# wangg12/mx-DeepIM

Measured on AMD Instinct MI355X. Metric: pose-refinements/sec (4 iters, 480x640), higher is better.
Workload: dtype f32

## Files before the change

### mx-deepim_amd/csrc/common.h

```cpp
#pragma once
#include <hip/hip_runtime.h>
#include <cstdarg>
#include <cstdio>
#include <cstdint>
#include <utility>

#include "../../include/deepim_hip.h"

namespace dim {

constexpr int kWave = 64;

char* err_buf();
int set_err(int code, const char* fmt, ...);

inline hipStream_t as_stream(void* s) { return reinterpret_cast<hipStream_t>(s); }

inline int check_launch(const char* what) {
  hipError_t e = hipGetLastError();
  if (e != hipSuccess) return set_err(DIM_ERR_LAUNCH, "%s: %s", what, hipGetErrorString(e));
  return DIM_OK;
}

inline int ceil_div(long a, long b) { return (int)((a + b - 1) / b); }
// ... 165 lines not shown
  for (int g = 1; g <= 8; g <<= 1) {
    if (count % g || wtile_lds_bytes(g, Q) > 65536) break;
    if (best == 0 || (long)outer * (count / g) >= 2048 || count / best > 65535) best = g;
  }
  return (best && count / best <= 65535 && outer <= 65535) ? best : 0;
}
template <bool TO_PACKED, typename PT>
inline void wtile_launch(const WTileArgs& a, int gx, int gy, hipStream_t st) {
  hipLaunchKernelGGL((weight_tile_kernel<TO_PACKED, PT>), dim3(gx, gy), dim3(256), wtile_lds_bytes(a.G, a.Q), st, a);
}
#endif

int conv2d_unpack_weight_slabs(const float* w_packed, int nslab, long slab_stride, float* w_oihw, int Cout, int CoutPad, int Cin, int KH, int KW,
                               float scale, int accumulate, void* stream);

struct WGemmArgs {
  const float* V;
  const float* U;
  float* M;
  int T, K, Cout, P;
  int nch;
  int NTN;
  int per, rem;
  unsigned v_bytes, u_bytes, m_bytes;
  FastDiv d_nch, d_P, d_NTN, d_MT;
  int G, BM, BN, tile;
  int MT;
  int plane_major;
  int dbg_plain;
  int wide_flush;
  const void* U3;
  unsigned u3_bytes;
  int split;
};
inline long wino_packed_with_split(long u_floats) { return u_floats + (u_floats * 3 + 1) / 2; }
int wino_split_weights(float* U, long chunks, int Cout, hipStream_t st);
void wino_set_split(int on);
int wino_get_split();
bool wino_gemm_split_has(int tile);
int wino_gemm_split_slots(int tile);
int wino_gemm_split_run(const WGemmArgs& a, hipStream_t st);
int wino_gemm_plan(WGemmArgs* plan, const float* V, const float* U, float* M, int T, int K, int Cout, int P, int tile);
int wino_gemm_run(const WGemmArgs& plan, bool zeroed, hipStream_t st);

#ifdef __HIPCC__
struct WCur {
  int ch, p, nt, mt;
};
__device__ __forceinline__ WCur wcur_decode(int chunk, const WGemmArgs& a) {
  WCur c;
  const unsigned item = fastdiv((unsigned)chunk, a.d_nch);
  c.ch = chunk - (int)item * a.nch;
  if (a.plane_major) {
    const unsigned t = fastdiv(item, a.d_NTN);
    c.nt = (int)(item - t * a.NTN);
    const unsigned p = fastdiv(t, a.d_MT);
    c.mt = (int)(t - p * a.MT);
    c.p = (int)p;
  } else {
    const unsigned t = fastdiv(item, a.d_P);
    c.p = (int)(item - t * a.P);
    const unsigned mt = fastdiv(t, a.d_NTN);
    c.nt = (int)(t - mt * a.NTN);
    c.mt = (int)mt;
  }
  return c;
}
__device__ __forceinline__ int wg_xcd_contiguous(int b, int G) {
  const int x = b & 7, j = b >> 3, q = G >> 3, r = G & 7;
  return (x < r ? x * (q + 1) : r * (q + 1) + (x - r) * q) + j;
}
__device__ __forceinline__ int wg_first_chunk(int w, const WGemmArgs& a) { return w * a.per + min(w, a.rem); }
__device__ __forceinline__ void wino_gemm_zero_tile(const WGemmArgs& a, int w) {
  const WCur c = wcur_decode(wg_first_chunk(w, a), a);
  if (c.ch == 0) return;
  const int ldc = a.P * a.Cout;
  float* base = a.M + (long)c.mt * a.BM * ldc + c.p * a.Cout + c.nt * a.BN;
  const int rows = min(a.BM, a.T - c.mt * a.BM);
  const int q = a.BN / 4;
  for (int idx = threadIdx.x; idx < rows * q; idx += 256) {
    const int r = idx / q, c4 = idx - r * q;
    *reinterpret_cast<float4*>(base + (long)r * ldc + c4 * 4) = make_float4(0.f, 0.f, 0.f, 0.f);
  }
}
#endif

}

#define DIM_REQUIRE(cond, ...)                                   \
  do {                                                           \
    if (!(cond)) return dim::set_err(DIM_ERR_ARG, __VA_ARGS__);  \
  } while (0)
```

### mx-deepim_amd/csrc/wino_gemm.hip

```cpp
#include <cstdlib>

#include "common.h"

namespace dim {

typedef float f32x16 __attribute__((ext_vector_type(16)));

__device__ __forceinline__ void wcur_advance(WCur& c, const WGemmArgs& a) {
  if (++c.ch == a.nch) {
    c.ch = 0;
    if (a.plane_major) {
      if (++c.nt == a.NTN) {
        c.nt = 0;
        if (++c.mt == a.MT) {
          c.mt = 0;
          ++c.p;
        }
      }
    } else if (++c.p == a.P) {
      c.p = 0;
      if (++c.nt == a.NTN) {
        c.nt = 0;
        ++c.mt;
      }
    }
  }
}
template <int BM, int BN, int WM, int WN>
__global__ __launch_bounds__(WM * WN * 64) __attribute__((amdgpu_waves_per_eu(BN == 256 || BM == 160 ? 2 : (BM == 96 ? 3 : 4), 8))) void wino_gemm_kernel(WGemmArgs a) {
  constexpr int BK = 32;
  constexpr int NT = WM * WN * 64;
  constexpr int RP = NT / 8;
  constexpr int LDK = BK + 4;
  constexpr int TM = BM / WM / 32;
  constexpr int TN = BN / WN / 32;
  constexpr int NSTG = BM / RP;
  constexpr int kTrLd = 32, kTrFloats = 16 * kTrLd;
  constexpr bool kWide = !(BM == 128 && BN == 128);
  static_assert(BM % RP == 0 && NSTG >= 2 && NSTG <= 5, "two to five staging loads per thread");

  extern __shared__ __attribute__((aligned(16))) float smem[];
  float* sA = smem;
  float* sTr = smem + 2 * BM * LDK;

  const int tid = threadIdx.x;
  const int lane = tid & 63;
  const int wave = tid >> 6;
  const int wm = wave / WN, wn = wave % WN;
  const int q = tid & 7;
  const int srow = tid >> 3;
  const int frow = lane & 31;
  const int khalf = lane >> 5;

  const int wg = a.plane_major ? wg_xcd_contiguous(blockIdx.x, a.G) : (int)blockIdx.x;
  const int c_begin = wg_first_chunk(wg, a);
  const int c_end = wg_first_chunk(wg + 1, a);

  const int RS = a.P * a.K;
  const int a_voff0 = (srow * RS + q * 4) * 4;
  const int a_vstep = RP * RS * 4;
  const __amdgpu_buffer_rsrc_t rv = __builtin_amdgcn_make_buffer_rsrc(const_cast<float*>(a.V), 0, a.v_bytes, 0x00020000);
  const __amdgpu_buffer_rsrc_t ru = __builtin_amdgcn_make_buffer_rsrc(const_cast<float*>(a.U), 0, a.u_bytes, 0x00020000);
  const __amdgpu_buffer_rsrc_t rm = __builtin_amdgcn_make_buffer_rsrc(a.M, 0, a.m_bytes, 0x00020000);
  const int wchunk_bytes = a.Cout * BK * 4;

  WCur L = wcur_decode(c_begin, a), Bc = L, C = L;

  float4 ra0, ra1, ra2, ra3, ra4;
#define W_LOAD_CHUNK(PF_OK)                                                            \
  {                                                                                    \
    const bool pf = (PF_OK);                                                           \
    const int mb = L.mt * BM;                                                          \
    const int soff = (int)((unsigned)(mb * RS + L.p * a.K + L.ch * BK) * 4u);          \
    ra0 = buf_load16_nt(rv, (pf && mb + srow < a.T) ? a_voff0 : -1, soff);             \
    ra1 = buf_load16_nt(rv, (pf && mb + srow + RP < a.T) ? a_voff0 + a_vstep : -1, soff);        \
    if constexpr (NSTG > 2) ra2 = buf_load16_nt(rv, (pf && mb + srow + 2 * RP < a.T) ? a_voff0 + 2 * a_vstep : -1, soff); \
    if constexpr (NSTG > 3) ra3 = buf_load16_nt(rv, (pf && mb + srow + 3 * RP < a.T) ? a_voff0 + 3 * a_vstep : -1, soff); \
    if constexpr (NSTG > 4) ra4 = buf_load16_nt(rv, (pf && mb + srow + 4 * RP < a.T) ? a_voff0 + 4 * a_vstep : -1, soff); \
    wcur_advance(L, a);                                                                \
  }
#define W_STORE_CHUNK(BUF)                                                             \
  {                                                                                    \
    float* dA = sA + (BUF) * BM * LDK;                                                 \
    *reinterpret_cast<float4*>(dA + srow * LDK + q * 4) = ra0;                         \
    *reinterpret_cast<float4*>(dA + (srow + RP) * LDK + q * 4) = ra1;                  \
    if constexpr (NSTG > 2) *reinterpret_cast<float4*>(dA + (srow + 2 * RP) * LDK + q * 4) = ra2; \
    if constexpr (NSTG > 3) *reinterpret_cast<float4*>(dA + (srow + 3 * RP) * LDK + q * 4) = ra3; \
    if constexpr (NSTG > 4) *reinterpret_cast<float4*>(dA + (srow + 4 * RP) * LDK + q * 4) = ra4; \
  }

  f32x16 acc[TM][TN];
#pragma unroll
  for (int i = 0; i < TM; ++i)
#pragma unroll
    for (int j = 0; j < TN; ++j)
#pragma unroll
      for (int r = 0; r < 16; ++r) acc[i][j][r] = 0.f;

  const int a_off = (wm * (BM / WM) + frow) * LDK + 4 * khalf;
  float4 fa[2][TM];
#define W_FRAG_READ(IDX, PA, S)                                                                                        \
  {                                                                                                                    \
    _Pragma("unroll") for (int i = 0; i < TM; ++i) fa[IDX][i] = *reinterpret_cast<const float4*>((PA) + 32 * i * LDK + 8 * (S)); \
  }
  float4 fbq[2][4][TN];
  const int bf_voff = ((wn * (BN / WN) + frow) * BK + 4 * khalf) * 4;
#define W_LOAD_BFRAG(SET, VALID)                                                                                       \
  {                                                                                                                    \
    const int bsoff = (VALID) ? (Bc.p * a.nch + Bc.ch) * wchunk_bytes + Bc.nt * BN * BK * 4 : 0;                        \
    _Pragma("unroll") for (int g = 0; g < 4; ++g) _Pragma("unroll") for (int j = 0; j < TN; ++j)                        \
      fbq[SET][g][j] = buf_load16(ru, bf_voff + (32 * j * BK + 8 * g) * 4, bsoff);                                      \
    wcur_advance(Bc, a);                                                                                               \
  }
#define W_MFMA_GROUP(IDX, SET, G)                                                                                      \
  {                                                                                                                    \
    __builtin_amdgcn_sched_barrier(0);                                                                                 \
    _Pragma("unroll") for (int i = 0; i < TM; ++i) _Pragma("unroll") for (int j = 0; j < TN; ++j) {                     \
      acc[i][j] = __builtin_amdgcn_mfma_f32_32x32x2f32(fa[IDX][i].x, fbq[SET][G][j].x, acc[i][j], 0, 0, 0);             \
      acc[i][j] = __builtin_amdgcn_mfma_f32_32x32x2f32(fa[IDX][i].y, fbq[SET][G][j].y, acc[i][j], 0, 0, 0);             \
      acc[i][j] = __builtin_amdgcn_mfma_f32_32x32x2f32(fa[IDX][i].z, fbq[SET][G][j].z, acc[i][j], 0, 0, 0);             \
      acc[i][j] = __builtin_amdgcn_mfma_f32_32x32x2f32(fa[IDX][i].w, fbq[SET][G][j].w, acc[i][j], 0, 0, 0);             \
    }                                                                                                                  \
    __builtin_amdgcn_sched_barrier(0);                                                                                 \
  }

  const int ldc = a.P * a.Cout;
  const int o_row = wm * (BM / WM) + 4 * khalf;
  const int o_col = wn * (BN / WN) + frow;
  const int o_voff = (o_row * ldc + o_col) * 4;
  bool whole = C.ch == 0;
#define W_FLUSH_CHECK(KCUR)                                                                                            \
  {                                                                                                                    \
    const bool item_end = C.ch == a.nch - 1;                                                                           \
    if (item_end || (KCUR) == c_end - 1) {                                                                             \
      const int mb = C.mt * BM;                                                                                        \
      const int cb = C.p * a.Cout + C.nt * BN;                                                                         \
      const int lim = a.T - mb;                                                                                        \
      int ov = o_voff, orow = o_row;  \
      asm volatile("" : "+v"(ov), "+v"(orow));                                                                         \
      const int soff = (int)((unsigned)(mb * ldc + cb) * 4u);                                                          \
      const bool plain = (whole && item_end) || a.dbg_plain;                                                           \
      if (kWide && plain && a.wide_flush) {                                                                            \
                                                        \
        float* sT = sTr + wave * kTrFloats;                                                                            \
        const int trow = lane >> 3, tc4 = (lane & 7) * 4;                                                              \
        _Pragma("unroll") for (int i = 0; i < TM; ++i) _Pragma("unroll") for (int j = 0; j < TN; ++j)                   \
          _Pragma("unroll") for (int h = 0; h < 2; ++h) {  \
            _Pragma("unroll") for (int r = 0; r < 8; ++r) sT[((r & 3) + 8 * (r >> 2) + 4 * khalf) * kTrLd + frow] = acc[i][j][8 * h + r]; \
            asm volatile("s_waitcnt lgkmcnt(0)" ::: "memory");                                                         \
             \
            const float4 t0 = *reinterpret_cast<const float4*>(sT + trow * kTrLd + tc4);                               \
            const float4 t1 = *reinterpret_cast<const float4*>(sT + (trow + 8) * kTrLd + tc4);                         \
            asm volatile("s_waitcnt lgkmcnt(0)" ::: "memory");                                                         \
            const int gr = wm * (BM / WM) + 32 * i + 16 * h + trow;                                                    \
            const int vo0 = (gr < lim) ? (gr * ldc + wn * (BN / WN) + 32 * j + tc4) * 4 : -1;                          \
            const int vo1 = (gr + 8 < lim) ? ((gr + 8) * ldc + wn * (BN / WN) + 32 * j + tc4) * 4 : -1;                \
            u32x4 u0, u1;                                                                                              \
            u0.x = __float_as_uint(t0.x); u0.y = __float_as_uint(t0.y); u0.z = __float_as_uint(t0.z); u0.w = __float_as_uint(t0.w); \
            u1.x = __float_as_uint(t1.x); u1.y = __float_as_uint(t1.y); u1.z = __float_as_uint(t1.z); u1.w = __float_as_uint(t1.w); \
            __builtin_amdgcn_raw_buffer_store_b128(u0, rm, vo0, soff, 2);                                              \
            __builtin_amdgcn_raw_buffer_store_b128(u1, rm, vo1, soff, 2);                                              \
            asm volatile("" ::: "memory");                                                                             \
          }                                                                                                            \
      } else                                                                                                           \
      _Pragma("unroll") for (int i = 0; i < TM; ++i) _Pragma("unroll") for (int j = 0; j < TN; ++j)                     \
        _Pragma("unroll") for (int r = 0; r < 16; ++r) {                                                               \
// ... 44 lines not shown
  }
#undef W_CHUNK_BODY
#undef W_FLUSH_CHECK
#undef W_MFMA_GROUP
#undef W_LOAD_BFRAG
#undef W_FRAG_READ
#undef W_STORE_CHUNK
#undef W_LOAD_CHUNK
}

__global__ __launch_bounds__(256) void wino_gemm_zero_kernel(WGemmArgs a) { wino_gemm_zero_tile(a, blockIdx.x + 1); }

static int g_wino_split = getenv("DIM_WINO_SPLIT") ? atoi(getenv("DIM_WINO_SPLIT")) : 1;
void wino_set_split(int on) { g_wino_split = on; }
int wino_get_split() { return g_wino_split; }
static int g_wino_cus = 0;
template <int BM, int BN, int WM, int WN>
static int wino_gemm_slots() {
  static int slots = 0;
  if (slots == 0) {
    int dev = 0, cus = 0, occ = 0;
    hipError_t e = hipGetDevice(&dev);
    if (e == hipSuccess) e = hipDeviceGetAttribute(&cus, hipDeviceAttributeMultiprocessorCount, dev);
    if (e == hipSuccess)
      e = hipOccupancyMaxActiveBlocksPerMultiprocessor(&occ, reinterpret_cast<const void*>(&wino_gemm_kernel<BM, BN, WM, WN>),
                                                       WM * WN * 64, (2 * BM * 36 + WM * WN * 512) * sizeof(float));
    if (e != hipSuccess || cus <= 0 || occ <= 0) return set_err(DIM_ERR_LAUNCH, "winograd gemm occupancy query: %s", hipGetErrorString(e));
    slots = cus * occ;
    g_wino_cus = cus;
  }
  return slots;
}

int wino_gemm_plan(WGemmArgs* plan, const float* V, const float* U, float* M, int T, int K, int Cout, int P, int tile) {
  if (tile == 5 && Cout % 256 != 0) tile = 4;
  if ((tile < 4 || tile > 7) || Cout % 128 != 0) tile = 3;
  const int BM = tile == 3 ? 64 : tile == 6 ? 160 : tile == 7 ? 96 : 128, BN = tile == 5 ? 256 : tile == 3 ? 64 : 128;
  DIM_REQUIRE(K % 32 == 0 && Cout % BN == 0 && T > 0, "winograd gemm: K %% 32 == 0 and Cout %% 64 == 0 required");
  const long MT = (T + BM - 1) / BM;
  const long items = MT * (Cout / BN) * P;
  DIM_REQUIRE(items * (K / 32) < (1L << 31) && (long)T * P * K * 4 < (1L << 32) && (long)T * P * Cout * 4 < (1L << 32) &&
                  (long)P * K * Cout * 4 < (1L << 31) && (long)BM * P * (K > Cout ? K : Cout) * 4 < (1L << 31),
              "winograd gemm: problem too large for 32-bit byte offsets (split the batch)");
  WGemmArgs a = {};
  a.V = V;
  a.U = U;
  a.M = M;
  a.T = T;
  a.K = K;
  a.Cout = Cout;
  a.P = P;
  a.nch = K / 32;
  a.NTN = Cout / BN;
  a.v_bytes = (unsigned)((long)T * P * K * 4);
  a.u_bytes = (unsigned)((long)P * K * Cout * 4);
  a.m_bytes = (unsigned)((long)T * P * Cout * 4);
  a.d_nch = make_fastdiv((unsigned)a.nch);
  a.d_P = make_fastdiv((unsigned)P);
  a.d_NTN = make_fastdiv((unsigned)a.NTN);
  a.MT = (int)MT;
  a.d_MT = make_fastdiv((unsigned)MT);
  static const int order = getenv("DIM_WINO_PLANE_MAJOR") ? atoi(getenv("DIM_WINO_PLANE_MAJOR")) : 1;
  a.plane_major = order;
  static const int dbg_plain = getenv("DIM_WINO_DBG_PLAIN") ? atoi(getenv("DIM_WINO_DBG_PLAIN")) : 0;
  a.dbg_plain = dbg_plain;
  static const int wide = getenv("DIM_WINO_WIDE_FLUSH") ? atoi(getenv("DIM_WINO_WIDE_FLUSH")) : 1;
  a.wide_flush = wide;
  a.BM = BM;
  a.BN = BN;
  a.tile = tile;
  a.split = g_wino_split && wino_gemm_split_has(tile) && (long)P * K * Cout * 6 < (1L << 31);
  a.U3 = U + (long)P * K * Cout;
  a.u3_bytes = (unsigned)((long)P * K * Cout * 6);
  if (a.split) a.plane_major = 1;
  const int slots = a.split ? wino_gemm_split_slots(tile) : tile == 5 ? wino_gemm_slots<128, 256, 2, 4>() : tile == 4 ? wino_gemm_slots<128, 128, 2, 4>()
                  : tile == 6 ? wino_gemm_slots<160, 128, 1, 4>() : tile == 7 ? wino_gemm_slots<96, 128, 1, 4>() : wino_gemm_slots<64, 64, 2, 2>();
  if (slots <= 0) return slots;
  a.G = items < slots ? (int)items : slots;
  static const int g_round = getenv("DIM_WINO_G_ROUND") ? atoi(getenv("DIM_WINO_G_ROUND")) : 1;
  if (g_wino_cus == 0) {
    int dev = 0;
    if (hipGetDevice(&dev) != hipSuccess || hipDeviceGetAttribute(&g_wino_cus, hipDeviceAttributeMultiprocessorCount, dev) != hipSuccess) g_wino_cus = 0;
  }
  if (g_round && g_wino_cus > 0 && a.G > g_wino_cus && a.G < slots) a.G = a.G / g_wino_cus * g_wino_cus;
  const long total = items * a.nch;
  a.per = (int)(total / a.G);
  a.rem = (int)(total % a.G);
  *plan = a;
  return DIM_OK;
}

template <int BM, int BN, int WM, int WN>
static int wino_gemm_launch(const WGemmArgs& a, hipStream_t st) {
  constexpr size_t lds = (2 * BM * 36 + WM * WN * 512) * sizeof(float);
  static_assert(lds <= 65536, "dynamic LDS of a plane-GEMM workgroup stays within 64 KB");
  hipLaunchKernelGGL((wino_gemm_kernel<BM, BN, WM, WN>), dim3(a.G), dim3(WM * WN * 64), lds, st, a);
  return check_launch("winograd_gemm");
}

int wino_gemm_run(const WGemmArgs& a, bool zeroed, hipStream_t st) {
  if (!zeroed && a.G > 1) hipLaunchKernelGGL(wino_gemm_zero_kernel, dim3(a.G - 1), dim3(256), 0, st, a);
  if (a.split) return wino_gemm_split_run(a, st);
  if (a.tile == 5) return wino_gemm_launch<128, 256, 2, 4>(a, st);
  if (a.tile == 4) return wino_gemm_launch<128, 128, 2, 4>(a, st);
  if (a.tile == 6) return wino_gemm_launch<160, 128, 1, 4>(a, st);
  if (a.tile == 7) return wino_gemm_launch<96, 128, 1, 4>(a, st);
  return wino_gemm_launch<64, 64, 2, 2>(a, st);
// ... 11 lines not shown
```

### mx-deepim_amd/csrc/wino_gemm_split.hip

```cpp
#include <cstdlib>

#include "common.h"

#ifndef DIM_SPLIT_EXP
#define DIM_SPLIT_EXP 0
#endif
#ifndef DIM_SPLIT_OPT
#define DIM_SPLIT_OPT 0
#endif

namespace dim {

typedef float f32x16 __attribute__((ext_vector_type(16)));
typedef float f32x4 __attribute__((ext_vector_type(4)));
typedef __bf16 bf16x8 __attribute__((ext_vector_type(8)));
typedef __bf16 bf16x4 __attribute__((ext_vector_type(4)));

struct Split4 {
  uint2 h, m, l;
};
__device__ __forceinline__ Split4 split3(const float4 v) {
  const f32x4 x = {v.x, v.y, v.z, v.w};
  const bf16x4 bh = __builtin_convertvector(x, bf16x4);
  const f32x4 r1 = x - __builtin_convertvector(bh, f32x4);
// ... 19 lines not shown
  const Split4 a = split3(src[0]), b = split3(src[1]);
  unsigned char* dst = U3 + (long)c * Cout * 192 + (long)(n >> 5) * 6144 + ((g >> 1) * 32 + (n & 31)) * 32 + (g & 1) * 16;
  *reinterpret_cast<uint4*>(dst) = make_uint4(a.h.x, a.h.y, b.h.x, b.h.y);
  *reinterpret_cast<uint4*>(dst + 2048) = make_uint4(a.m.x, a.m.y, b.m.x, b.m.y);
  *reinterpret_cast<uint4*>(dst + 4096) = make_uint4(a.l.x, a.l.y, b.l.x, b.l.y);
}

int wino_split_weights(float* U, long chunks, int Cout, hipStream_t st) {
  if (Cout % 32 != 0) return DIM_OK;
  const long total = chunks * Cout * 4;
  unsigned char* U3 = reinterpret_cast<unsigned char*>(U + chunks * Cout * 32);
  hipLaunchKernelGGL(wino_split_weights_kernel, dim3((unsigned)((total + 255) / 256)), dim3(256), 0, st, U, U3, total, Cout,
                     make_fastdiv((unsigned)Cout));
  return check_launch("winograd_split_weights");
}

#if DIM_SPLIT_EXP & 128
__device__ unsigned long long g_split_stamps[1024 * 8 * 11];
#endif
#if (DIM_SPLIT_EXP & 128) && defined(__HIP_DEVICE_COMPILE__)
#define S_STAMP(K)                                                                     \
  {                                                                                    \
    unsigned long long t_;                                                             \
    __builtin_amdgcn_sched_barrier(0);                                                 \
    asm volatile("s_memtime %0\n\ts_waitcnt lgkmcnt(0)" : "=s"(t_)::"memory");         \
    __builtin_amdgcn_sched_barrier(0);                                                 \
    seg[K] += t_ - tprev;                                                              \
    tprev = t_;                                                                        \
  }
#else
#define S_STAMP(K)
#endif

__device__ __forceinline__ void wscur_advance(WCur& c, const WGemmArgs& a) {
  if (++c.ch == a.nch) {
    c.ch = 0;
    if (++c.nt == a.NTN) {
      c.nt = 0;
      if (++c.mt == a.MT) {
        c.mt = 0;
        ++c.p;
      }
    }
  }
}

template <int BM, int WN>
__global__ __launch_bounds__(WN * 64) __attribute__((amdgpu_waves_per_eu(2, 2))) void wino_gemm_split_kernel(WGemmArgs a) {
  constexpr int BK = 32;
  constexpr int NT = WN * 64;
  constexpr int BN = 32 * WN;
  constexpr int TM = BM / 32;
  constexpr int RP = NT / 8;
  constexpr int NSTG = BM / RP;
  constexpr int PL = BM * 64;
  constexpr int kTrLd = 32, kTrFloats = 16 * kTrLd;
  constexpr int kMAux = ((DIM_SPLIT_OPT & 2) || BM == 96) ? 0 : 2;
  static_assert(BM % 32 == 0 && BM % RP == 0 && RP % 32 == 0 && NSTG >= 2 && NSTG <= 4, "two to four staging loads per thread");

  extern __shared__ __attribute__((aligned(16))) unsigned char smem_split[];
  unsigned char* sA = smem_split;
  float* sTr = reinterpret_cast<float*>(smem_split + 2 * 3 * PL);

  const int tid = threadIdx.x;
  const int lane = tid & 63;
  const int wave = tid >> 6;
  const int q = tid & 7;
  const int srow = tid >> 3;
  const int frow = lane & 31;
  const int khalf = lane >> 5;

  const int wg = wg_xcd_contiguous(blockIdx.x, a.G);
  const int c_begin = wg_first_chunk(wg, a);
  const int c_end = wg_first_chunk(wg + 1, a);

  const int RS = a.P * a.K;
  const int a_voff0 = (srow * RS + q * 4) * 4;
  const int a_vstep = RP * RS * 4;
  const __amdgpu_buffer_rsrc_t rv = __builtin_amdgcn_make_buffer_rsrc(const_cast<float*>(a.V), 0, a.v_bytes, 0x00020000);
  const __amdgpu_buffer_rsrc_t ru = __builtin_amdgcn_make_buffer_rsrc(const_cast<void*>(a.U3), 0, a.u3_bytes, 0x00020000);
  const __amdgpu_buffer_rsrc_t rm = __builtin_amdgcn_make_buffer_rsrc(a.M, 0, a.m_bytes, 0x00020000);
  const int wchunk_bytes = a.Cout * 192;

  WCur L = wcur_decode(c_begin, a), Bc = L, C = L;

  float4 rav[2][NSTG];
#define S_LOAD_PREP(PF_OK)                                                             \
  const bool l_pf = (PF_OK);                                                           \
  const int l_mb = L.mt * BM;                                                          \
  const int l_soff = (int)((unsigned)(l_mb * RS + L.p * a.K + L.ch * BK) * 4u);        \
  wscur_advance(L, a);
#define S_LOAD_ISSUE(RSET)                                                             \
  _Pragma("unroll") for (int ps = 0; ps < NSTG; ++ps)                                   \
    rav[RSET][ps] = buf_load16_nt(rv, (l_pf && l_mb + srow + ps * RP < a.T) ? a_voff0 + ps * a_vstep : -1, l_soff);
  const int st_off = srow * 64 + ((((q >> 1) ^ (srow >> 2)) & 3) << 4) + (q & 1) * 8;
#define S_STORE_ONE(DA, R, PASS)                                                       \
  {                                                                                    \
    const Split4 s = split3(R);                                                        \
    *reinterpret_cast<uint2*>((DA) + (PASS) * RP * 64) = s.h;                          \
    *reinterpret_cast<uint2*>((DA) + PL + (PASS) * RP * 64) = s.m;                     \
    *reinterpret_cast<uint2*>((DA) + 2 * PL + (PASS) * RP * 64) = s.l;                 \
  }
#define S_STORE_CHUNK(BUF, RSET)                                                       \
  {                                                                                    \
    unsigned char* dA = sA + (BUF) * 3 * PL + st_off;                                  \
    _Pragma("unroll") for (int ps = 0; ps < NSTG; ++ps) S_STORE_ONE(dA, rav[RSET][ps], ps) \
  }

  f32x16 acc[TM];
#pragma unroll
  for (int i = 0; i < TM; ++i)
#pragma unroll
    for (int r = 0; r < 16; ++r) acc[i][r] = 0.f;

  const int fr_off = frow * 64 + (((khalf ^ (frow >> 2)) & 3) << 4);
  bf16x8 fa[TM][3];
#define S_FRAG_READ(T, PA, S)                                                                                          \
  {                                                                                                                    \
    _Pragma("unroll") for (int i = 0; i < TM; ++i)                                                                      \
      fa[i][T] = *reinterpret_cast<const bf16x8*>((PA) + (T) * PL + i * 2048 + (fr_off ^ (32 * (S))));                 \
  }
  bf16x8 fb[2][3][2];
  const int bf_voff = wave * 6144 + frow * 32 + khalf * 16;
#define S_BFRAG_PREP(VALID)                                                                                            \
  const int b_soff = (VALID) ? (Bc.p * a.nch + Bc.ch) * wchunk_bytes + Bc.nt * BN * 192 : 0;                            \
  wscur_advance(Bc, a);
#define S_BFRAG_ISSUE(SET)                                                                                             \
  _Pragma("unroll") for (int t = 0; t < 3; ++t) _Pragma("unroll") for (int s = 0; s < 2; ++s) {                         \
    const float4 v = buf_load16(ru, bf_voff + (t * 2 + s) * 1024, b_soff);                                             \
    fb[SET][t][s] = __builtin_bit_cast(bf16x8, v);                                                                     \
  }
  static constexpr int kTA[2][6] = {{2, 0, 1, 1, 0, 0}, {2, 1, 1, 0, 0, 0}};
  static constexpr int kTB[2][6] = {{0, 2, 1, 0, 1, 0}, {0, 1, 0, 2, 1, 0}};
  f32x4 sp_x, sp_r;
  bf16x4 sp_h, sp_m, sp_l;

  const int ldc = a.P * a.Cout;
  const int o_row = 4 * khalf;
  const int o_col = wave * 32 + frow;
  const int o_voff = (o_row * ldc + o_col) * 4;
  bool whole = C.ch == 0;
#define S_FLUSH_CHECK(KCUR)                                                                                            \
  {                                                                                                                    \
    const bool item_end = C.ch == a.nch - 1;                                                                           \
    if (item_end || (KCUR) == c_end - 1) {                                                                             \
      const int mb = C.mt * BM;                                                                                        \
      const int cb = C.p * a.Cout + C.nt * BN;                                                                         \
      const int lim = a.T - mb;                                                                                        \
      int ov = o_voff, orow = o_row;                                                                                   \
      asm volatile("" : "+v"(ov), "+v"(orow));                                                                         \
      const int soff = (int)((unsigned)(mb * ldc + cb) * 4u);                                                          \
      const bool plain = (whole && item_end) || a.dbg_plain;                                                           \
      if (plain && a.wide_flush) {                                                                                     \
        float* sT = sTr + wave * kTrFloats;                                                                            \
        const int trow = lane >> 3, tc4 = (lane & 7) * 4;                                                              \
        _Pragma("unroll") for (int i = 0; i < TM; ++i) _Pragma("unroll") for (int h = 0; h < 2; ++h) {                  \
                \
          if constexpr (!(DIM_SPLIT_OPT & 16))                                                                         \
          _Pragma("unroll") for (int r = 0; r < 8; ++r) sT[((r & 3) + 8 * (r >> 2) + 4 * khalf) * kTrLd + frow] = acc[i][8 * h + r]; \
          float4 t0, t1;                                                                                               \
          if constexpr (DIM_SPLIT_OPT & 16) {                            \
            t0 = make_float4(acc[i][8 * h], acc[i][8 * h + 1], acc[i][8 * h + 2], acc[i][8 * h + 3]);                  \
            t1 = make_float4(acc[i][8 * h + 4], acc[i][8 * h + 5], acc[i][8 * h + 6], acc[i][8 * h + 7]);              \
          } else {                                                                                                     \
            t0 = *reinterpret_cast<const float4*>(sT + trow * kTrLd + tc4);                                            \
            t1 = *reinterpret_cast<const float4*>(sT + (trow + 8) * kTrLd + tc4);                                      \
          }                                                                                                            \
          const int gr = 32 * i + 16 * h + trow;                                                                       \
          const int vo0 = (gr < lim) ? (gr * ldc + wave * 32 + tc4) * 4 : -1;                                          \
          const int vo1 = (gr + 8 < lim) ? ((gr + 8) * ldc + wave * 32 + tc4) * 4 : -1;                                \
          u32x4 u0, u1;                                                                                                \
          u0.x = __float_as_uint(t0.x); u0.y = __float_as_uint(t0.y); u0.z = __float_as_uint(t0.z); u0.w = __float_as_uint(t0.w); \
          u1.x = __float_as_uint(t1.x); u1.y = __float_as_uint(t1.y); u1.z = __float_as_uint(t1.z); u1.w = __float_as_uint(t1.w); \
          if constexpr (DIM_SPLIT_OPT & 8) {                                             \
            if constexpr (!(DIM_SPLIT_OPT & 64)) asm volatile("" ::"v"(u0), "v"(u1));                                  \
          } else {                                                                                                     \
            __builtin_amdgcn_raw_buffer_store_b128(u0, rm, vo0, soff, kMAux);                                          \
// ... 188 lines not shown
```

### mx-deepim_amd/csrc/winograd.hip

```cpp
#include <cstdlib>

#include "common.h"

namespace dim {

__device__ __forceinline__ float4 f4add(float4 a, float4 b) { return make_float4(a.x + b.x, a.y + b.y, a.z + b.z, a.w + b.w); }
__device__ __forceinline__ float4 f4sub(float4 a, float4 b) { return make_float4(a.x - b.x, a.y - b.y, a.z - b.z, a.w - b.w); }

__global__ __launch_bounds__(256) void wino_input_kernel(const float* __restrict__ x, float* __restrict__ V, int N, int H, int W, int C,
                                                         int in_cstride, int th, int tw, FastDiv div_cq, FastDiv div_tw, FastDiv div_th) {
  const unsigned idx = blockIdx.x * 256u + threadIdx.x;
  const unsigned CQ = C >> 2;
  const unsigned T = (unsigned)N * th * tw;
  const unsigned t = fastdiv(idx, div_cq);
  if (t >= T) return;
  const unsigned cq = idx - t * CQ;
  const unsigned r = fastdiv(t, div_tw);
  const unsigned tx = t - r * tw;
  const unsigned n = fastdiv(r, div_th);
  const unsigned ty = r - n * th;
  const int y0 = 2 * (int)ty - 1, x0 = 2 * (int)tx - 1;
  const float* base = x + (long)n * H * W * in_cstride + cq * 4;
  float4 d[4][4];
#pragma unroll
// ... 89 lines not shown
    Gg[0][j] = g[j];
    Gg[1][j] = 0.5f * (g[j] + g[3 + j] + g[6 + j]);
    Gg[2][j] = 0.5f * (g[j] - g[3 + j] + g[6 + j]);
    Gg[3][j] = g[6 + j];
  }
  const long per_k = (long)Cin * Cout;
  float* o = wp + ((long)(ci >> 5) * Cout + co) * 32 + (ci & 31);
#pragma unroll
  for (int i = 0; i < 4; ++i) {
    o[(i * 4 + 0) * per_k] = Gg[i][0];
    o[(i * 4 + 1) * per_k] = 0.5f * (Gg[i][0] + Gg[i][1] + Gg[i][2]);
    o[(i * 4 + 2) * per_k] = 0.5f * (Gg[i][0] - Gg[i][1] + Gg[i][2]);
    o[(i * 4 + 3) * per_k] = Gg[i][2];
  }
}

constexpr int kWino4Vec = 2;

template <int VEC>
struct WinoVec {
  typedef float type __attribute__((ext_vector_type(VEC)));
};

#define DIM_WINO4_BT(O, D, S)                                                          \
  {                                                                                    \
    O[0 * S] = D[0] + 1.5f * D[1] - 2.f * D[2] - 1.5f * D[3] + D[4];                    \
    O[1 * S] = D[4] - D[1] - 2.5f * D[2] - 0.5f * D[3];                                 \
    O[2 * S] = D[4] + D[1] + 0.5f * D[2] - 2.5f * D[3];                                 \
    O[3 * S] = D[4] - 0.5f * D[1] - D[2] + 0.5f * D[3];                                 \
    O[4 * S] = D[4] + 2.f * D[1] - D[2] - 2.f * D[3];                                   \
    O[5 * S] = D[1] + 1.5f * D[2] - 2.f * D[3] - 1.5f * D[4] + D[5];                    \
  }

template <int VEC, int S>
__global__ __launch_bounds__(256) void wino4_input_kernel(const float* __restrict__ x, float* __restrict__ V, int N, int H, int W, int C,
                                                          int in_cstride, int th, int tw, FastDiv div_cq, FastDiv div_tw, FastDiv div_th,
                                                          unsigned nblk, WGemmArgs plan) {
#pragma clang fp contract(fast)
  typedef typename WinoVec<VEC>::type vf;
  if (blockIdx.x >= nblk) {
    wino_gemm_zero_tile(plan, (int)(blockIdx.x - nblk) + 1);
    return;
  }
  const unsigned idx = (unsigned)wg_xcd_contiguous((int)blockIdx.x, (int)nblk) * 256u + threadIdx.x;
  const unsigned CT = C * S * S;
  const unsigned CQ = CT / VEC;
  const unsigned T = (unsigned)N * th * tw;
  const unsigned t = fastdiv(idx, div_cq);
  if (t >= T) return;
  const unsigned cq = idx - t * CQ;
  const unsigned r = fastdiv(t, div_tw);
  const unsigned tx = t - r * tw;
  const unsigned n = fastdiv(r, div_th);
  const unsigned ty = r - n * th;
  const int y0 = 4 * (int)ty - 1, x0 = 4 * (int)tx - 1;
  const unsigned cc = cq * VEC;
  const unsigned ph = S == 1 ? 0u : (unsigned)(cc >= (unsigned)C) + (unsigned)(cc >= 2u * C) + (unsigned)(cc >= 3u * C);
  const int py = ph >> 1, px = ph & 1;
  const float* base = x + (long)n * H * W * in_cstride + (cc - ph * C);
  vf tmp[36];
#pragma unroll
  for (int b = 0; b < 6; ++b) {
    const int xx = S * (x0 + b) + px;
    const bool okx = (unsigned)xx < (unsigned)W;
    const int xc = okx ? xx : 0;
    vf d[6];
#pragma unroll
    for (int a = 0; a < 6; ++a) {
      const int yy = S * (y0 + a) + py;
      const bool ok = okx && (unsigned)yy < (unsigned)H;
      const int yc = (unsigned)yy < (unsigned)H ? yy : 0;
      vf v = *reinterpret_cast<const vf*>(base + ((long)yc * W + xc) * in_cstride);
      d[a] = ok ? v : (vf)(0.f);
    }
    vf* o = tmp + b;
    DIM_WINO4_BT(o, d, 6)
  }
  const long plane = CT;
  float* out = V + (long)t * 36 * CT + cc;
#pragma unroll
  for (int a = 0; a < 6; ++a) {
    vf o[6];
    const vf* d = tmp + 6 * a;
    DIM_WINO4_BT(o, d, 1)
#pragma unroll
    for (int b = 0; b < 6; ++b) __builtin_nontemporal_store(o[b], reinterpret_cast<vf*>(out + (a * 6 + b) * plane));
  }
}

#define DIM_WINO4_AT(O, M, S)                                       \
  {                                                                 \
    const vf s1 = M[1] + M[2], d1 = M[1] - M[2];                    \
    O[0 * S] = M[0] + s1 + M[3] + M[4];                             \
    O[1 * S] = d1 + 2.f * M[3] - 0.5f * M[4];                       \
    O[2 * S] = s1 + 4.f * M[3] + 0.25f * M[4];                      \
    O[3 * S] = d1 + 8.f * M[3] - 0.125f * M[4] + M[5];              \
  }

template <int VEC, int S>
__global__ __launch_bounds__(256) void wino4_output_kernel(const float* __restrict__ M, const float* __restrict__ bias, float* __restrict__ y,
                                                           int N, int H, int W, int C, int out_cstride, int out_coff, int th, int tw,
                                                           float slope, FastDiv div_cq, FastDiv div_tw, FastDiv div_th) {
#pragma clang fp contract(fast)
  typedef typename WinoVec<VEC>::type vf;
  const unsigned idx = blockIdx.x * 256u + threadIdx.x;
  const unsigned CT = C * S * S;
  const unsigned CQ = CT / VEC;
  const unsigned T = (unsigned)N * th * tw;
  const unsigned t = fastdiv(idx, div_cq);
  if (t >= T) return;
  const unsigned cq = idx - t * CQ;
  const unsigned r = fastdiv(t, div_tw);
  const unsigned tx = t - r * tw;
  const unsigned n = fastdiv(r, div_th);
  const unsigned ty = r - n * th;
  const long plane = CT;
  const unsigned cc = cq * VEC;
  const unsigned ph = S == 1 ? 0u : (unsigned)(cc >= (unsigned)C) + (unsigned)(cc >= 2u * C) + (unsigned)(cc >= 3u * C);
  const int py = ph >> 1, px = ph & 1;
// ... 229 lines not shown

int dim_winograd_dgrad_pack_weight(const float* w_oihw, float* w_packed, int Cout, int Cin, int m, void* stream) {
  DIM_REQUIRE(w_oihw && w_packed, "null weight pointer");
  DIM_REQUIRE(m == 2 || m == 4, "output tile m must be 2 or 4");
  DIM_REQUIRE(Cout % 32 == 0 && Cin % 64 == 0, "Cout %% 32 == 0 and Cin %% 64 == 0 required");
  long total = (long)Cout * Cin;
  if (m == 2)
    hipLaunchKernelGGL(wino_pack_weight_kernel<true>, dim3(ceil_div(total, 256)), dim3(256), 0, as_stream(stream), w_oihw, w_packed, Cin, Cout);
  else
    hipLaunchKernelGGL(wino4_pack_weight_kernel<true>, dim3(ceil_div(total, 256)), dim3(256), 0, as_stream(stream), w_oihw, w_packed, Cin, Cout);
  int rc = check_launch("winograd_dgrad_pack_weight");
  return rc != DIM_OK ? rc : wino_split_weights(w_packed, (long)(m + 2) * (m + 2) * (Cout / 32), Cin, as_stream(stream));
}

static int winograd_slice(const float* x, const float* w_packed, const float* bias, float* y, float* workspace, int N, int H, int W, int Cin,
                          int in_cstride, int Cout, int out_cstride, int out_coff, float slope, int tile, int m, int S, void** events4,
                          void* stream) {
  const int Ho = S == 1 ? H : (H + 1) / 2, Wo = S == 1 ? W : (W + 1) / 2;
  const int CT = Cin * S * S;
  const int th = (Ho + m - 1) / m, tw = (Wo + m - 1) / m;
  const int nk = (m + 2) * (m + 2);
  const long T = (long)N * th * tw;
  float* V = workspace;
  float* M = workspace + nk * T * CT;
  hipStream_t st = as_stream(stream);
  const FastDiv dtw = make_fastdiv((unsigned)tw), dth = make_fastdiv((unsigned)th);
#define DIM_WINO_EVENT(I)                                                                  \
  if (events4 && events4[I]) {                                                             \
    hipError_t e = hipEventRecord(reinterpret_cast<hipEvent_t>(events4[I]), st);           \
    if (e != hipSuccess) return set_err(DIM_ERR_LAUNCH, "hipEventRecord: %s", hipGetErrorString(e)); \
  }
  if (tile == 0) tile = (Cout % 128 == 0 && T >= 1024) ? 4 : 3;
  WGemmArgs plan;
  int rc = wino_gemm_plan(&plan, V, w_packed, M, (int)T, CT, Cout, nk, tile);
  if (rc != DIM_OK) return rc;
  DIM_WINO_EVENT(0)
  const unsigned nblk = (unsigned)ceil_div(T * (CT / kWino4Vec), 256);
  if (m == 2)
    hipLaunchKernelGGL(wino_input_kernel, dim3(ceil_div(T * (Cin / 4), 256)), dim3(256), 0, st, x, V, N, H, W, Cin, in_cstride, th, tw,
                       make_fastdiv((unsigned)(Cin / 4)), dtw, dth);
  else if (S == 1)
    hipLaunchKernelGGL((wino4_input_kernel<kWino4Vec, 1>), dim3(nblk + plan.G - 1), dim3(256), 0, st, x, V, N, H, W, Cin, in_cstride, th, tw,
                       make_fastdiv((unsigned)(CT / kWino4Vec)), dtw, dth, nblk, plan);
  else
    hipLaunchKernelGGL((wino4_input_kernel<kWino4Vec, 2>), dim3(nblk + plan.G - 1), dim3(256), 0, st, x, V, N, H, W, Cin, in_cstride, th, tw,
                       make_fastdiv((unsigned)(CT / kWino4Vec)), dtw, dth, nblk, plan);
  rc = check_launch("winograd_input");
  if (rc != DIM_OK) return rc;
  DIM_WINO_EVENT(1)
  rc = wino_gemm_run(plan, m == 4, st);
  if (rc != DIM_OK) return rc;
  DIM_WINO_EVENT(2)
  if (m == 2)
    hipLaunchKernelGGL(wino_output_kernel, dim3(ceil_div(T * (Cout / 4), 256)), dim3(256), 0, st, M, bias, y, N, Ho, Wo, Cout, out_cstride,
                       out_coff, th, tw, slope, make_fastdiv((unsigned)(Cout / 4)), dtw, dth);
  else
    hipLaunchKernelGGL((wino4_output_kernel<kWino4Vec, 1>), dim3(ceil_div(T * (Cout / kWino4Vec), 256)), dim3(256), 0, st, M, bias, y, N, Ho, Wo,
                       Cout, out_cstride, out_coff, th, tw, slope, make_fastdiv((unsigned)(Cout / kWino4Vec)), dtw, dth);
  rc = check_launch("winograd_output");
  DIM_WINO_EVENT(3)
#undef DIM_WINO_EVENT
  return rc;
}

static int winograd_impl(const float* x, const float* w_packed, const float* bias, float* y, float* workspace, int N, int H, int W, int Cin,
                         int in_cstride, int Cout, int out_cstride, int out_coff, float slope, int tile, int m, int S, void** events4,
                         void* stream) {
  if (N == 0) return DIM_OK;
  DIM_REQUIRE(x && w_packed && y && workspace, "null pointer");
  DIM_REQUIRE(m == 2 || m == 4, "output tile m must be 2 or 4");
  DIM_REQUIRE(Cin % 32 == 0 && Cout % 64 == 0, "Cin %% 32 == 0 and Cout %% 64 == 0 required");
  if (in_cstride == 0) in_cstride = Cin;
  if (out_cstride == 0) out_cstride = Cout;
  DIM_REQUIRE(in_cstride >= Cin && in_cstride % 4 == 0 && out_cstride >= out_coff + Cout && out_cstride % 4 == 0 && out_coff % 4 == 0,
              "channel strides / offsets must be multiples of 4 and cover the channels");
  const int Ho = S == 1 ? H : (H + 1) / 2, Wo = S == 1 ? W : (W + 1) / 2;
  const long ns = wino_slice_images((long)((Ho + m - 1) / m) * ((Wo + m - 1) / m), (m + 2) * (m + 2), (long)Cin * S * S, Cout);
  DIM_REQUIRE(ns > 0, "one image alone exceeds the 32-bit offsets of the plane GEMMs");
// ... 150 lines not shown
```

### mx-deepim_amd/deepim/symbols/deepIM_flownet.py

```python
import os

import numpy as np
import torch

from lib.hip import ops

ENCODER = [
    ("flow_conv1", 64, 7, 2, 3),
    ("conv2", 128, 5, 2, 2),
    ("conv3", 256, 5, 2, 2),
    ("conv3_1", 256, 3, 1, 1),
    ("conv4", 512, 3, 2, 1),
    ("conv4_1", 512, 3, 1, 1),
    ("conv5", 512, 3, 2, 1),
    ("conv5_1", 512, 3, 1, 1),
    ("conv6", 1024, 3, 2, 1),
    ("conv6_1", 1024, 3, 1, 1),
]


WINO_M_DEFAULT = {}
BF16_BIG_TILE = int(os.environ.get("DIM_BF16_BIG_TILE", "4"))
BF16_PATCH = os.environ.get("DIM_BF16_PATCH", "") != "0"
BF16_PATCH_S2_KERNELS = {"": (5,), "1": (), "2": (3, 5)}.get(os.environ.get("DIM_BF16_PATCH", ""), ())
# ... 236 lines not shown
                    self.packed[n] = ops.conv_small_cout_pack_weight(self.params[n + "_weight"])
            self.flow6 = torch.empty((B, 8, 10, 2), dtype=torch.float32, device=d)
            self.concat2 = torch.zeros((B, 15, 20, ops.pad64(1026)), dtype=torch.float32, device=d)
            self.flow5 = torch.empty((B, 15, 20, 2), dtype=torch.float32, device=d)
            self.concat3 = torch.zeros((B, 30, 40, ops.pad64(770)), dtype=torch.float32, device=d)
            self.flow4 = torch.empty((B, 30, 40, 2), dtype=torch.float32, device=d)
            self.mask4 = torch.empty((B, 30, 40, 1), dtype=torch.float32, device=d)
            self.zoom_flow = torch.empty((B, 2, H, W), dtype=torch.float32, device=d)
            self.flow_est = torch.empty((B, 2, H, W), dtype=torch.float32, device=d)
            self.zoom_mask_prob = torch.empty((B, 1, H, W), dtype=torch.float32, device=d)
            self.mask_pred = torch.empty((B, 1, H, W), dtype=torch.float32, device=d)
        self.fc6 = torch.empty((B, 1, 1, 256), dtype=torch.float32, device=d)
        self.fc7 = torch.empty((B, 256), dtype=torch.float32, device=d)
        self.se3 = torch.empty((B, 7), dtype=torch.float32, device=d)
        self.zoom_factor = torch.empty((B, 4), dtype=torch.float32, device=d)
        self.bbox_obs = torch.empty((B, 4), dtype=torch.int32, device=d)
        self.bbox_ren = torch.empty((B, 4), dtype=torch.int32, device=d)
        self.status = torch.zeros((B,), dtype=torch.int32, device=d)
        torch.cuda.synchronize(d)

    def pack_conv(self, w_oihw):
        return ops.conv2d_pack_weight(w_oihw, as_bf16=self.bf16)

    def pack_deconv(self, w_iohw):
        return ops.deconv4x4s2_pack_weight(w_iohw, as_bf16=self.bf16)

    @staticmethod
    def _wino_tile(cout, tiles, planes=36):
        return int(ops.lib().dim_winograd_gemm_tile_planes(int(cout), int(tiles), int(planes)))

    @staticmethod
    def _wino_info(m, S, tile, tiles, cin, cout, x_floats, y_floats, planes=None):
        planes, K = planes or (m + 2) ** 2, cin * S * S
        return dict(winograd=True, wino_m=m, wino_tile=tile, wino_planes=planes, wino_rows=tiles, wino_k=K,
                    wino_flops=2 * planes * tiles * K * cout, wino_gemm_bytes=4 * planes * (tiles * K + K * cout + tiles * cout),
                    wino_in_bytes=4 * (x_floats + planes * tiles * K), wino_out_bytes=4 * (planes * tiles * cout + y_floats),
                    wino_in_kernel="dim::wino_input_kernel" if m == 2 else "dim::wino4_input_kernel<2, %d>" % S,
                    wino_out_kernel="dim::wino_output_kernel" if m == 2 else "dim::wino4_output_kernel<2>")

    def zoom(self, batch, bbox_ren=None, nchw_out=None, bbox_obs=None, src_pose=None, status=None):
        if self.zoom_from_masks:
            if bbox_obs is None:
                bbox_obs = ops.mask_bbox(batch["mask_observed"], 0.3, out=self.bbox_obs)
            if bbox_ren is None:
                bbox_ren = ops.mask_bbox(batch["mask_rendered"], 0.2, out=self.bbox_ren)
        else:
            bbox_obs = ops.mask_bbox(batch["image_observed"], 0.01, mode=1, means3=self.plane_means, out=self.bbox_obs)
            bbox_ren = ops.mask_bbox(batch["image_rendered"], 0.01, mode=1, means3=self.plane_means, out=self.bbox_ren)
        ops.zoom_factor(bbox_obs, bbox_ren, batch["src_pose"] if src_pose is None else src_pose, self.K, self.H, self.W,
                        out=self.zoom_factor, status=self.status if status is None else status)
        return self.net_input(batch, nchw_out=nchw_out)

    def net_input(self, batch, nchw_out=None):
        if self.input_mode == 0:
            ops.zoom_net_input(batch["image_observed"], batch["image_rendered"], batch["mask_observed"], batch["mask_rendered"],
                               self.zoom_factor, self.plane_means, X=self.X, nchw_out=nchw_out)
        elif self.input_mode == 1:
            ops.zoom_net_input_ex(batch["image_observed"], batch["image_rendered"], None, None, self.zoom_factor, self.plane_means, 1, X=self.X)
        else:
            ops.zoom_net_input_ex(batch["image_observed"], batch["image_rendered"], batch["depth_observed"], batch["depth_rendered"],
                                  self.zoom_factor, self.plane_means, 2, X=self.X)
            if self.input_mode == 3:
                ops.zoom_net_input_ex(batch["image_observed"], batch["image_rendered"], batch["mask_observed"], batch["mask_rendered"],
                                      self.zoom_factor, self.plane_means, 3, X=self.X2)
        return self.X

    def encoder(self, X=None, events=None):
        x = self.X if X is None else X
        for name, cout, k, s, p in ENCODER:
            if name in self.wino:
# ... 123 lines not shown
```

Baseline: 1650.

## Skip structurally zero phase blocks in stride-2 Winograd F(4,3) GEMM

For stride-2 convolutions decomposed into four phase sub-kernels, some Winograd planes are identically zero for certain phases. A per-plane phase mask now makes the GEMM iterators skip those K-chunks, recounts each workgroup's chunk range, and stops the input transform from writing the unused V entries. The goal is to cut wasted MFMA work and V/U memory traffic. In exchange the chunk-walking logic gets more complex, and load balance shifts because work is still split by raw chunk counts.

```diff
diff --git a/mx-deepim_amd/csrc/common.h b/mx-deepim_amd/csrc/common.h
--- a/mx-deepim_amd/csrc/common.h
+++ b/mx-deepim_amd/csrc/common.h
@@ -221,6 +221,7 @@
   const void* U3;
   unsigned u3_bytes;
   int split;
+  int skip5, q;
 };
 inline long wino_packed_with_split(long u_floats) { return u_floats + (u_floats * 3 + 1) / 2; }
 int wino_split_weights(float* U, long chunks, int Cout, hipStream_t st);
@@ -229,14 +230,41 @@
 bool wino_gemm_split_has(int tile);
 int wino_gemm_split_slots(int tile);
 int wino_gemm_split_run(const WGemmArgs& a, hipStream_t st);
-int wino_gemm_plan(WGemmArgs* plan, const float* V, const float* U, float* M, int T, int K, int Cout, int P, int tile);
+int wino_gemm_plan(WGemmArgs* plan, const float* V, const float* U, float* M, int T, int K, int Cout, int P, int tile, int skip5 = 0);
 int wino_gemm_run(const WGemmArgs& plan, bool zeroed, hipStream_t st);
 
 #ifdef __HIPCC__
 struct WCur {
   int ch, p, nt, mt;
+  int m;
 };
-__device__ __forceinline__ WCur wcur_decode(int chunk, const WGemmArgs& a) {
+__host__ __device__ __forceinline__ int wino5_phase_mask(int p) { return (p >= 30 ? 0x3 : 0xF) & (p % 6 == 5 ? 0x5 : 0xF); }
+__device__ __forceinline__ int wcur_snap(int ch, int m, const WGemmArgs& a) {
+  const int q = a.q;
+  const int ph = (ch >= q) + (ch >= 2 * q) + (ch >= 3 * q);
+  if ((m >> ph) & 1) return ch;
+  const int r = m >> (ph + 1);
+  return r ? (ph + 1 + __builtin_ctz(r)) * q : a.nch;
+}
+__device__ __forceinline__ void wcur_advance_pm(WCur& c, const WGemmArgs& a) {
+  ++c.ch;
+  if (c.m != 0xF) c.ch = wcur_snap(c.ch, c.m, a);
+  if (c.ch >= a.nch) {
+    c.ch = 0;
+    if (++c.nt == a.NTN) {
+      c.nt = 0;
+      if (++c.mt == a.MT) {
+        c.mt = 0;
+        ++c.p;
+        if (a.skip5) c.m = wino5_phase_mask(c.p);
+      }
+    }
+  }
+}
+__device__ __forceinline__ bool wcur_item_end(const WCur& c, const WGemmArgs& a) {
+  return (c.m != 0xF ? wcur_snap(c.ch + 1, c.m, a) : c.ch + 1) >= a.nch;
+}
+__device__ __forceinline__ WCur wcur_decode_raw(int chunk, const WGemmArgs& a) {
   WCur c;
   const unsigned item = fastdiv((unsigned)chunk, a.d_nch);
   c.ch = chunk - (int)item * a.nch;
@@ -255,6 +283,29 @@
   }
   return c;
 }
+__device__ __forceinline__ WCur wcur_decode(int chunk, const WGemmArgs& a) {
+  WCur c = wcur_decode_raw(chunk, a);
+  c.m = a.skip5 ? wino5_phase_mask(c.p) : 0xF;
+  if (c.m != 0xF) {
+    c.ch = wcur_snap(c.ch, c.m, a) - 1;
+    wcur_advance_pm(c, a);
+  }
+  return c;
+}
+__device__ __forceinline__ int wcur_count(int begin, int end, const WGemmArgs& a) {
+  if (!a.skip5) return end - begin;
+  int n = 0;
+  for (int v = begin; v < end;) {
+    const unsigned item = fastdiv((unsigned)v, a.d_nch);
+    const int base = (int)item * a.nch, lo = v - base, hi = min(end - base, a.nch);
+    const int m = wino5_phase_mask((int)fastdiv(fastdiv(item, a.d_NTN), a.d_MT));
+#pragma unroll
+    for (int ph = 0; ph < 4; ++ph)
+      if ((m >> ph) & 1) n += max(0, min(hi, (ph + 1) * a.q) - max(lo, ph * a.q));
+    v = base + a.nch;
+  }
+  return n;
+}
 __device__ __forceinline__ int wg_xcd_contiguous(int b, int G) {
   const int x = b & 7, j = b >> 3, q = G >> 3, r = G & 7;
   return (x < r ? x * (q + 1) : r * (q + 1) + (x - r) * q) + j;
diff --git a/mx-deepim_amd/csrc/wino_gemm.hip b/mx-deepim_amd/csrc/wino_gemm.hip
--- a/mx-deepim_amd/csrc/wino_gemm.hip
+++ b/mx-deepim_amd/csrc/wino_gemm.hip
@@ -7,6 +7,7 @@
 typedef float f32x16 __attribute__((ext_vector_type(16)));
 
 __device__ __forceinline__ void wcur_advance(WCur& c, const WGemmArgs& a) {
+  if (a.plane_major) return wcur_advance_pm(c, a);
   if (++c.ch == a.nch) {
     c.ch = 0;
     if (a.plane_major) {
@@ -53,8 +54,9 @@
   const int khalf = lane >> 5;
 
   const int wg = a.plane_major ? wg_xcd_contiguous(blockIdx.x, a.G) : (int)blockIdx.x;
-  const int c_begin = wg_first_chunk(wg, a);
-  const int c_end = wg_first_chunk(wg + 1, a);
+  const int r_begin = wg_first_chunk(wg, a);
+  const int c_begin = 0, c_end = wcur_count(r_begin, wg_first_chunk(wg + 1, a), a);
+  if (c_end == 0) return;
 
   const int RS = a.P * a.K;
   const int a_voff0 = (srow * RS + q * 4) * 4;
@@ -64,7 +66,7 @@
   const __amdgpu_buffer_rsrc_t rm = __builtin_amdgcn_make_buffer_rsrc(a.M, 0, a.m_bytes, 0x00020000);
   const int wchunk_bytes = a.Cout * BK * 4;
 
-  WCur L = wcur_decode(c_begin, a), Bc = L, C = L;
+  WCur L = wcur_decode(r_begin, a), Bc = L, C = L;
 
   float4 ra0, ra1, ra2, ra3, ra4;
 #define W_LOAD_CHUNK(PF_OK)                                                            \
@@ -131,7 +133,7 @@
   bool whole = C.ch == 0;
 #define W_FLUSH_CHECK(KCUR)                                                                                            \
   {                                                                                                                    \
-    const bool item_end = C.ch == a.nch - 1;                                                                           \
+    const bool item_end = wcur_item_end(C, a);                                                                         \
     if (item_end || (KCUR) == c_end - 1) {                                                                             \
       const int mb = C.mt * BM;                                                                                        \
       const int cb = C.p * a.Cout + C.nt * BN;                                                                         \
@@ -242,7 +244,7 @@
   return slots;
 }
 
-int wino_gemm_plan(WGemmArgs* plan, const float* V, const float* U, float* M, int T, int K, int Cout, int P, int tile) {
+int wino_gemm_plan(WGemmArgs* plan, const float* V, const float* U, float* M, int T, int K, int Cout, int P, int tile, int skip5) {
   if (tile == 5 && Cout % 256 != 0) tile = 4;
   if ((tile < 4 || tile > 7) || Cout % 128 != 0) tile = 3;
   const int BM = tile == 3 ? 64 : tile == 6 ? 160 : tile == 7 ? 96 : 128, BN = tile == 5 ? 256 : tile == 3 ? 64 : 128;
@@ -282,7 +284,10 @@
   a.split = g_wino_split && wino_gemm_split_has(tile) && (long)P * K * Cout * 6 < (1L << 31);
   a.U3 = U + (long)P * K * Cout;
   a.u3_bytes = (unsigned)((long)P * K * Cout * 6);
-  if (a.split) a.plane_major = 1;
+  DIM_REQUIRE(!skip5 || (P == 36 && a.nch % 4 == 0), "winograd gemm: skipping zero phase blocks needs 36 planes and K = 4 phases of whole chunks");
+  a.skip5 = skip5;
+  a.q = a.nch / 4;
+  if (a.split || skip5) a.plane_major = 1;
   const int slots = a.split ? wino_gemm_split_slots(tile) : tile == 5 ? wino_gemm_slots<128, 256, 2, 4>() : tile == 4 ? wino_gemm_slots<128, 128, 2, 4>()
                   : tile == 6 ? wino_gemm_slots<160, 128, 1, 4>() : tile == 7 ? wino_gemm_slots<96, 128, 1, 4>() : wino_gemm_slots<64, 64, 2, 2>();
   if (slots <= 0) return slots;
diff --git a/mx-deepim_amd/csrc/wino_gemm_split.hip b/mx-deepim_amd/csrc/wino_gemm_split.hip
--- a/mx-deepim_amd/csrc/wino_gemm_split.hip
+++ b/mx-deepim_amd/csrc/wino_gemm_split.hip
@@ -75,18 +75,7 @@
 #define S_STAMP(K)
 #endif
 
-__device__ __forceinline__ void wscur_advance(WCur& c, const WGemmArgs& a) {
-  if (++c.ch == a.nch) {
-    c.ch = 0;
-    if (++c.nt == a.NTN) {
-      c.nt = 0;
-      if (++c.mt == a.MT) {
-        c.mt = 0;
-        ++c.p;
-      }
-    }
-  }
-}
+__device__ __forceinline__ void wscur_advance(WCur& c, const WGemmArgs& a) { wcur_advance_pm(c, a); }
 
 template <int BM, int WN>
 __global__ __launch_bounds__(WN * 64) __attribute__((amdgpu_waves_per_eu(2, 2))) void wino_gemm_split_kernel(WGemmArgs a) {
@@ -114,8 +103,9 @@
   const int khalf = lane >> 5;
 
   const int wg = wg_xcd_contiguous(blockIdx.x, a.G);
-  const int c_begin = wg_first_chunk(wg, a);
-  const int c_end = wg_first_chunk(wg + 1, a);
+  const int r_begin = wg_first_chunk(wg, a);
+  const int c_begin = 0, c_end = wcur_count(r_begin, wg_first_chunk(wg + 1, a), a);
+  if (c_end == 0) return;
 
   const int RS = a.P * a.K;
   const int a_voff0 = (srow * RS + q * 4) * 4;
@@ -125,7 +115,7 @@
   const __amdgpu_buffer_rsrc_t rm = __builtin_amdgcn_make_buffer_rsrc(a.M, 0, a.m_bytes, 0x00020000);
   const int wchunk_bytes = a.Cout * 192;
 
-  WCur L = wcur_decode(c_begin, a), Bc = L, C = L;
+  WCur L = wcur_decode(r_begin, a), Bc = L, C = L;
 
   float4 rav[2][NSTG];
 #define S_LOAD_PREP(PF_OK)                                                             \
@@ -185,7 +175,7 @@
   bool whole = C.ch == 0;
 #define S_FLUSH_CHECK(KCUR)                                                                                            \
   {                                                                                                                    \
-    const bool item_end = C.ch == a.nch - 1;                                                                           \
+    const bool item_end = wcur_item_end(C, a);                                                                         \
     if (item_end || (KCUR) == c_end - 1) {                                                                             \
       const int mb = C.mt * BM;                                                                                        \
       const int cb = C.p * a.Cout + C.nt * BN;                                                                         \
diff --git a/mx-deepim_amd/csrc/winograd.hip b/mx-deepim_amd/csrc/winograd.hip
--- a/mx-deepim_amd/csrc/winograd.hip
+++ b/mx-deepim_amd/csrc/winograd.hip
@@ -145,7 +145,8 @@
     O[5 * S] = D[1] + 1.5f * D[2] - 2.f * D[3] - 1.5f * D[4] + D[5];                    \
   }
 
-template <int VEC, int S>
+
+template <int VEC, int S, bool FWD5 = false>
 __global__ __launch_bounds__(256) void wino4_input_kernel(const float* __restrict__ x, float* __restrict__ V, int N, int H, int W, int C,
                                                           int in_cstride, int th, int tw, FastDiv div_cq, FastDiv div_tw, FastDiv div_th,
                                                           unsigned nblk, WGemmArgs plan) {
@@ -197,7 +198,9 @@
     const vf* d = tmp + 6 * a;
     DIM_WINO4_BT(o, d, 1)
 #pragma unroll
-    for (int b = 0; b < 6; ++b) __builtin_nontemporal_store(o[b], reinterpret_cast<vf*>(out + (a * 6 + b) * plane));
+    for (int b = 0; b < 6; ++b)
+      if (!FWD5 || ((a < 5 || py == 0) && (b < 5 || px == 0)))
+        __builtin_nontemporal_store(o[b], reinterpret_cast<vf*>(out + (a * 6 + b) * plane));
   }
 }
 
@@ -493,7 +496,7 @@
   }
   if (tile == 0) tile = (Cout % 128 == 0 && T >= 1024) ? 4 : 3;
   WGemmArgs plan;
-  int rc = wino_gemm_plan(&plan, V, w_packed, M, (int)T, CT, Cout, nk, tile);
+  int rc = wino_gemm_plan(&plan, V, w_packed, M, (int)T, CT, Cout, nk, tile, S == 2);
   if (rc != DIM_OK) return rc;
   DIM_WINO_EVENT(0)
   const unsigned nblk = (unsigned)ceil_div(T * (CT / kWino4Vec), 256);
@@ -504,7 +507,7 @@
     hipLaunchKernelGGL((wino4_input_kernel<kWino4Vec, 1>), dim3(nblk + plan.G - 1), dim3(256), 0, st, x, V, N, H, W, Cin, in_cstride, th, tw,
                        make_fastdiv((unsigned)(CT / kWino4Vec)), dtw, dth, nblk, plan);
   else
-    hipLaunchKernelGGL((wino4_input_kernel<kWino4Vec, 2>), dim3(nblk + plan.G - 1), dim3(256), 0, st, x, V, N, H, W, Cin, in_cstride, th, tw,
+    hipLaunchKernelGGL((wino4_input_kernel<kWino4Vec, 2, true>), dim3(nblk + plan.G - 1), dim3(256), 0, st, x, V, N, H, W, Cin, in_cstride, th, tw,
                        make_fastdiv((unsigned)(CT / kWino4Vec)), dtw, dth, nblk, plan);
   rc = check_launch("winograd_input");
   if (rc != DIM_OK) return rc;
diff --git a/mx-deepim_amd/deepim/symbols/deepIM_flownet.py b/mx-deepim_amd/deepim/symbols/deepIM_flownet.py
--- a/mx-deepim_amd/deepim/symbols/deepIM_flownet.py
+++ b/mx-deepim_amd/deepim/symbols/deepIM_flownet.py
@@ -292,10 +292,11 @@
     @staticmethod
     def _wino_info(m, S, tile, tiles, cin, cout, x_floats, y_floats, planes=None):
         planes, K = planes or (m + 2) ** 2, cin * S * S
+        pk = 121 * (K // 4) if S == 2 else planes * K
         return dict(winograd=True, wino_m=m, wino_tile=tile, wino_planes=planes, wino_rows=tiles, wino_k=K,
-                    wino_flops=2 * planes * tiles * K * cout, wino_gemm_bytes=4 * planes * (tiles * K + K * cout + tiles * cout),
-                    wino_in_bytes=4 * (x_floats + planes * tiles * K), wino_out_bytes=4 * (planes * tiles * cout + y_floats),
-                    wino_in_kernel="dim::wino_input_kernel" if m == 2 else "dim::wino4_input_kernel<2, %d>" % S,
+                    wino_flops=2 * pk * tiles * cout, wino_gemm_bytes=4 * (tiles * pk + pk * cout + planes * tiles * cout),
+                    wino_in_bytes=4 * (x_floats + tiles * pk), wino_out_bytes=4 * (planes * tiles * cout + y_floats),
+                    wino_in_kernel="dim::wino_input_kernel" if m == 2 else "dim::wino4_input_kernel<2, %d, %s>" % (S, "true" if S == 2 else "false"),
                     wino_out_kernel="dim::wino_output_kernel" if m == 2 else "dim::wino4_output_kernel<2>")
 
     def zoom(self, batch, bbox_ren=None, nchw_out=None, bbox_obs=None, src_pose=None, status=None):
```

Result: faster. 1683 (median of 6 runs) (+2.0%).
